# mgholamikn/PoseGen

Measured on AMD Instinct MI355X. Metric: rendered rays/sec (512x512, 64 samples/ray), higher is better.
Workload: dtype bf16

## Files before the change

posegen_amd/csrc/pg_api.hip:

```cpp
#include <hip/hip_runtime.h>

#include <cstdarg>
#include <cstdio>
#include <cstdlib>
#include <chrono>
#include <cstring>
#include <algorithm>
#include <mutex>
#include <thread>
#include <new>
#include <utility>
#include <vector>

#include "../../include/posegen_hip.h"
#include "pg_device.h"
#include "pg_handle.h"
#include "pg_pack.h"

extern "C" {
int pg_launch_eval16(const pgd::EvalArgs* a, int fp16, int framecode, int grid, void* stream);
int pg_launch_eval16r(const pgd::EvalArgs* a, int fp16, int framecode, int onchip, int grid, void* stream);
int pg_launch_ray_records(const pgd::RecArgs* a, int fp16, int framecode, int n_cu, void* stream);
int pg_eval16_points_per_pass(void);
int pg_eval16_wgs_per_cu(void);
// ... 130 lines not shown
    }
}

enum Form {
    F_DIRECT16,
    F_REC16,
    F_ONCHIP16,
    F_C2,
    F_COMP_DIRECT,
    F_COMP_REC,
    F_COMP_ONCHIP,
    F_KMAJOR,
    F_COUNT
};

struct Switches {
    bool view_fact = true;
    bool comp_kernel = true;
    bool comp_rec = true;
    bool evalc2 = true;
    int onchip = PG_ONCHIP_AUTO;
};
const Switches& switches() {
    static const Switches sw = [] {
        auto off = [](const char* name) { const char* e = std::getenv(name); return e && e[0] == '0'; };
        Switches s;
        s.view_fact = !off("POSEGEN_VIEW_FACT");
        s.comp_kernel = !off("POSEGEN_COMP_KERNEL");
        s.comp_rec = !off("POSEGEN_COMP_REC");
        s.evalc2 = !off("POSEGEN_EVALC2");
        const char* e = std::getenv("POSEGEN_ONCHIP");
        s.onchip = e && e[0] == '0' ? PG_ONCHIP_RECORDS : e && e[0] == '2' ? PG_ONCHIP_ALWAYS : PG_ONCHIP_AUTO;
        return s;
    }();
    return sw;
}

struct CallFacts {
    int prec;
    int S;
    long long pose_stride;
    bool fc;
    bool points, pnoise;
    bool dbg; int dbg_stage;
    int onchip_mode;
};

// ... 273 lines not shown
    a.S = S;
    a.n_codes = ns.n_codes;
    a.tau_v = h->tau[0];
    a.tau_d = h->tau[1];
    a.dbg_stage = dbg_stage;
    a.far_skip = h->far_skip ? 1 : 0;
    const int pts = fi.points_per_pass();
    if (!points && S < pts / (MAXR - 1))
        return pg_fail(h, PG_EINVAL, "N_samples=%d too small: the fused kernel needs >= %d samples per ray", S, pts / (MAXR - 1));
    const long long iters = (a.n_points + pts - 1) / pts;
    a.n_iters = (int)iters;
    static const long long wg_cap = [] { const char* e = std::getenv("POSEGEN_MAX_WG"); return e ? std::atoll(e) : 0ll; }();
    long long max_wg = (long long)h->n_cu * fi.wgs_per_cu();
    if (wg_cap > 0 && wg_cap < max_wg) max_wg = wg_cap;
    const int grid = (int)(iters < max_wg ? iters : max_wg);
    hipEvent_t e0 = nullptr, e1 = nullptr;
    auto get = [&](hipEvent_t& ev) {
        if (!h->ev_free.empty()) { ev = h->ev_free.back(); h->ev_free.pop_back(); return hipSuccess; }
        return hipEventCreate(&ev);
    };
    if (y_bytes) {
        pgd::RecArgs ra{};
        ra.rays = rays; ra.skts = skts; ra.cams = cams; ra.codes = a.codes; ra.wy = a.wy;
        ra.rec_ab = const_cast<float*>(a.rec_ab); ra.rec_y = const_cast<uint8_t*>(a.rec_y);
        ra.pose_stride = pose_stride; ra.n_rays = (int)n; ra.n_codes = ns.n_codes;
        ra.z = z; ra.S = S;
        hipEvent_t x0 = nullptr, x1 = nullptr;
        if (h->profiling) { PG_HIP(h, get(x0)); PG_HIP(h, get(x1)); PG_HIP(h, hipEventRecord(x0, static_cast<hipStream_t>(stream))); }
        const int er = form == F_COMP_REC ? pg_launch_ray_records_c(&ra, fc, h->n_cu, stream) : pg_launch_ray_records(&ra, prec == PG_PREC_FP16, fc, h->n_cu, stream);
        if (h->profiling) {
// ... 483 lines not shown

int pg_debug_widen_views(const float* view_w, int64_t rows, int64_t cols, int framecode_ch, float* out, int64_t cap,
                         int64_t* out_n) {
    if (!view_w) return pg_fail(nullptr, PG_EINVAL, "pg_debug_widen_views: null argument");
    if (framecode_ch != 0 && framecode_ch != FC_CH) return pg_fail(nullptr, PG_EINVAL, "pg_debug_widen_views: frame code 0 or 16");
    if (rows != VW || cols != W + CH_D0 + framecode_ch)
        return pg_fail(nullptr, PG_EINVAL, "pg_debug_widen_views: view weight [%lld,%lld], expected [%d,%d]", (long long)rows,
                       (long long)cols, VW, W + CH_D0 + framecode_ch);
    const int64_t need = (int64_t)VW * (W + CH_D + framecode_ch);
    if (out_n) *out_n = need;
    if (out) {
        if (cap < need) return pg_fail(nullptr, PG_EINVAL, "pg_debug_widen_views: buffer too small");
        widen_view_w(view_w, framecode_ch, out);
    }
    return PG_OK;
}

int pg_debug_pack_vy(const float* const* tensors, const int64_t* shapes, int n_tensors, int framecode_ch,
                     int precision, uint8_t* out, int64_t cap, int64_t* out_bytes) {
    if (!tensors || !shapes || n_tensors != 24) return pg_fail(nullptr, PG_EINVAL, "pg_debug_pack_vy: need 24 tensors");
    NetState ns;
    host_copy(ns, tensors, shapes, framecode_ch);
    pg_config cfg{};
    cfg.framecode_ch = framecode_ch;
    std::vector<uint8_t> vy;
    if (precision == PG_PREC_FP16C) {
        std::vector<float> f;
        pgpack::pack_vyc(tensors_of(ns, cfg), framecode_ch > 0, f);
        vy.resize(f.size() * sizeof(float));
        std::memcpy(vy.data(), f.data(), vy.size());
// ... 796 lines not shown
```

posegen_amd/csrc/pg_device.h:

```cpp
#pragma once
#include <hip/hip_runtime.h>

#include <atomic>

#include "pg_program.h"

namespace pgd {
using namespace pgl;

typedef __attribute__((ext_vector_type(8))) __bf16 bf16x8;
typedef __attribute__((ext_vector_type(8))) _Float16 f16x8;
typedef __attribute__((ext_vector_type(16))) float f32x16;

struct EvalArgs {
    const float* rays;
    const float* z;
    const float* pts;
    const float* pnoise;
    const float* skts;
    const float* cams;
    const float* codes;
    const uint8_t* wstream;
    const uint8_t* wy;
    const float* rec_ab;
    const uint8_t* rec_y;
    const float* bias;
    const float* cutoff;
    float* raw;
    float* dbg;
    long long pose_stride;
    long long n_points;
    int n_rays;
    int S;
    int n_codes;
    int n_iters;
    float tau_v, tau_d;
    int dbg_stage;
    int far_skip;
};

struct RecArgs {
    const float* rays;
    const float* skts;
    const float* cams;
    const float* codes;
    const uint8_t* wy;
    float* rec_ab;
    uint8_t* rec_y;
    const float* z;
    long long pose_stride;
    int n_rays;
    int n_codes;
    int S;
};

template <const int (&P)[24]>
__device__ __forceinline__ int perm_dev(int s) {
    constexpr unsigned long long lo = [] { unsigned long long v = 0; for (int i = 0; i < 12; ++i) v |= (unsigned long long)P[i] << (5 * i); return v; }();
    constexpr unsigned long long hi = [] { unsigned long long v = 0; for (int i = 0; i < 12; ++i) v |= (unsigned long long)P[12 + i] << (5 * i); return v; }();
    return (int)(((s < 12 ? lo : hi) >> (5 * (s < 12 ? s : s - 12))) & 31);
}
__device__ __forceinline__ int slot_joint_dev(int s) { return perm_dev<PERM16>(s); }
__device__ __forceinline__ int slotc_joint_dev(int s) { return perm_dev<PERMC>(s); }

inline hipError_t ensure_lds_attr(const void* fn, int bytes, std::atomic<unsigned long long>& done) {
    int dev = 0;
    hipError_t e = hipGetDevice(&dev);
    if (e != hipSuccess) return e;
// ... 379 lines not shown
```

posegen_amd/csrc/pg_eval16r.hip:

```cpp
#ifndef PG_PREFETCH
#define PG_PREFETCH 1
#endif
#ifndef PG_PIPE_H
#define PG_PIPE_H 4
#endif
#include <type_traits>

#include "pg_eval16_common.h"

#ifndef PG_REC_POLICY
#define PG_REC_POLICY ""
#endif

namespace pgd {

typedef __attribute__((ext_vector_type(4))) float f32x4;

template <typename V> struct Op16;
template <> struct Op16<bf16x8> {
    static __device__ __forceinline__ f32x4 mfma(bf16x8 a, bf16x8 b, f32x4 c) {
        return __builtin_amdgcn_mfma_f32_16x16x32_bf16(a, b, c, 0, 0, 0);
    }
};
template <> struct Op16<f16x8> {
// ... 270 lines not shown
    const float tlv = a.tau_v * 1.4426950408889634f, tld = a.tau_d * 1.4426950408889634f;
    if (tid < 48) cut[tid] = -a.cutoff[(tid < J ? 0 : J) + slot_joint_dev(tid < J ? tid : tid - J)] * (tid < J ? tlv : tld);
    else if (tid < 72) {
        const int jt = slot_joint_dev(tid - 48);
        const float far = fmaxf(a.cutoff[jt] + 24.0f / tlv, a.cutoff[J + jt] + 24.0f / tld);
        cut[tid] = far * far;
    }
    if (OC) {
        if (!PP) for (int i = tid; i < J * 12; i += NTHR) reinterpret_cast<float*>(smem + LDSR_SK)[i] = a.skts[slot_joint_dev(i / 12) * 16 + i % 12];
        for (int i = tid; i < MAXR_F * REC_Y_BYTES / 16; i += NTHR) reinterpret_cast<uint4*>(smem + LDSR_Y)[i] = make_uint4(0u, 0u, 0u, 0u);
    }
#if defined(PG_YOUNG_PRIO)
    if (wave >= NWAVE / 2) __builtin_amdgcn_s_setprio(PG_YOUNG_PRIO);
#endif
    const unsigned bbase = lds_addr_of(bias) + 16 * g;
    const long long step = (long long)PTS * gridDim.x;
    const int dq = __builtin_amdgcn_readfirstlane((int)(step / a.S)), dr = __builtin_amdgcn_readfirstlane((int)(step % a.S));
    long long p0 = (long long)blockIdx.x * PTS;
    int r0 = __builtin_amdgcn_readfirstlane((int)(p0 / a.S));
    int off0 = __builtin_amdgcn_readfirstlane((int)(p0 - (long long)r0 * a.S));
    if (OC) {
        lds_barrier();
        if (tid < MAXR_F * J) {
            const int k = tid / J, sl = tid - k * J;
            const long long ray = min((long long)r0 + k, (long long)a.n_rays - 1);
            const float* skr = PP ? a.skts + ray * a.pose_stride + slot_joint_dev(sl) * 16 : sk_lds + sl * 12;
            ab_row(skr, a.rays + ray * 11, a.z[ray * a.S], a.z[ray * a.S + a.S - 1],
                   reinterpret_cast<float4*>(smem + LDSR_AB + k * REC_AB_BYTES + sl * 32));
        }
    } else if ((int)blockIdx.x < a.n_iters && wave < LDS_AB_BYTES / 1024)
        dma_piece(rec_ab + (long long)r0 * REC_AB_BYTES + wave * 1024, lds0 + LDSR_AB + wave * 1024, lane16);
    if (OC && FC) {
        const float* ytab = reinterpret_cast<const float*>(a.wy);
        for (int idx = tid; idx < MAXR_F * VW; idx += NTHR) {
            const int k = idx / VW, o = idx - k * VW;
// ... 17 lines not shown
#endif
    st.start((uint32_t)gmask);

    float nx_z[2] = {0.0f, 0.0f};
#define PG_PREFETCH_Z(itn)                                                                         \
    do {                                                                                           \
        const long long p0n_ = (long long)(itn) * PTS + wave * 32 + col;                           \
        nx_z[0] = a.z[min(p0n_, a.n_points - 1)];                                                  \
        nx_z[1] = a.z[min(p0n_ + 16, a.n_points - 1)];                                             \
    } while (0)
    if ((int)blockIdx.x < a.n_iters) PG_PREFETCH_Z(blockIdx.x);

#if defined(PG_STAMPS)
    unsigned long long stamps[12];
#endif
    for (int it = blockIdx.x; it < a.n_iters; it += gridDim.x) {
        PG_STAMP(0);
        int lane_p = lane;
        asm volatile("" : "+v"(lane_p));
        const int g_p = lane_p >> 4;
        const int last = (int)min((long long)PTS - 1, a.n_points - 1 - p0);
        const int S1 = a.S, S2 = 2 * a.S, S3 = 3 * a.S, S4 = 4 * a.S;
        auto ray_of = [&](int t) { return (t >= S1) + (t >= S2) + (t >= S3) + (t >= S4); };
        const int nrm1 = ray_of(off0 + last);
        int myr[2];
        float zz[2];
        const float* abp[2];
#pragma unroll
        for (int c = 0; c < 2; ++c) {
            const int i = wave * 32 + 16 * c + col;
            myr[c] = min(ray_of(off0 + i), nrm1);
            zz[c] = nx_z[c];
            abp[c] = opaque_ptr(reinterpret_cast<const float*>(smem + LDSR_AB + abuf * LDS_AB_BYTES + myr[c] * REC_AB_BYTES) + JG * g_p * 8);
        }
        const int itn = min(it + (int)gridDim.x, a.n_iters - 1);
        int off0n = off0 + dr, r0n = r0 + dq;
        if (off0n >= a.S) { off0n -= a.S; ++r0n; }
        const float* cutd = opaque_ptr(cut + J + JG * g_p);
        const QFromAB q0{abp[0], zz[0]}, q1{abp[1], zz[1]};
        float cutv[JG];
#pragma unroll
        for (int jj = 0; jj < JG; ++jj) cutv[jj] = cut[JG * g_p + jj];
        int farmask = 0;
#if !defined(PG_NO_FAR_SKIP)
        {
            const float* far2 = opaque_ptr(cut + 2 * J + JG * g_p);
#pragma unroll
            for (int jj = 0; jj < JG; ++jj) {
                float ax, ay, az, bx, by, bz;
                q0(jj, ax, ay, az);
                q1(jj, bx, by, bz);
                const bool near = fminf(ax * ax + ay * ay + az * az, bx * bx + by * by + bz * bz) < far2[jj];
                if (__builtin_amdgcn_ballot_w64(near) == 0ull) farmask |= 1 << jj;
            }
            farmask = __builtin_amdgcn_readfirstlane(a.far_skip ? farmask : 0);
        }
#endif
        if (CNT && lane == 0) {
            if (wave == 0) { atomicAdd(reinterpret_cast<unsigned*>(a.dbg), 1u); atomicAdd(reinterpret_cast<unsigned*>(a.dbg) + 1, (unsigned)__builtin_popcount(gmask)); }
            atomicAdd(reinterpret_cast<unsigned*>(a.dbg) + 2, (unsigned)__builtin_popcount(farmask));
        }
        auto fetch_records = [&]() {
            if (OC) {
                const long long rn = min((long long)r0n, (long long)a.n_rays - 1);
                if (wave == 0) dma_dwords(a.rays, (uint32_t)(min(rn * 11 + lane_p, (long long)a.n_rays * 11 - 1) * 4), lds0 + LDSR_STAGE);
                else if (wave == 1) {
                    const long long ray = min(rn + min(lane_p >> 1, MAXR_F - 1), (long long)a.n_rays - 1);
                    dma_dwords(a.z, (uint32_t)((ray * a.S + ((lane_p & 1) ? a.S - 1 : 0)) * 4), lds0 + LDSR_STAGE + 256);
                } else if (FC && wave == 2 && a.cams)
                    dma_dwords(a.cams, (uint32_t)(min(rn + min(lane_p, MAXR_F - 1), (long long)a.n_rays - 1) * 4), lds0 + LDSR_STAGE + 512);
                return;
// ... 77 lines not shown
                    if (u == PG_R_BIAS_AT && o + 1 < NT16) bp.fetch(o + 1);
                }
            }
            x_segment16<V>(acc, st, abp[0], abp[1], zz[0], zz[1], cutv, tlv, farmask, gmask, [] {});
#pragma unroll
            for (int u = 0; u < HU16; ++u)
#pragma unroll
                for (int c = 0; c < 2; ++c) fb[u][c] = relu_pack16<V>(acc[2 * u][c], acc[2 * u + 1][c], true);
        }
        PG_STAMP(4);
        hidden_layer16<V>(fb, fa, st, bbase, BS_LAYER0 + 6 * NT16, C_L6);
        hidden_layer16<V>(fa, fb, st, bbase, BS_LAYER0 + 7 * NT16, C_L6 + CH);
        PG_STAMP(5);
        int gmask_n = 0;
#if !defined(PG_NO_FAR_SKIP)
        gmask_n = pass_far_mask(smem + LDSR_AB + (abuf ^ 1) * LDS_AB_BYTES, rays_of_pass(p0 + step, off0n),
                                opaque_ptr(cut + 2 * J + JG * g_p), g_p, lane_p & 15);
        if (!a.far_skip) gmask_n = 0;
#endif
        st.nx_mask = (uint32_t)gmask_n;
        float sigma[2];
        V fg[NTV16 / 2][2];
        APipe<V> pv;
        {
            f32x4 vacc[NTV16][2];
            constexpr int TAV = pgp::R::U_AV;
            static_assert(BS_VIEWF == BS_ALPHA + 1 && BS_RGB == BS_VIEWF + NTV16, "alpha, view and rgb bias tiles are consecutive");
            BiasPipe bp(bbase, BS_ALPHA);
            bp.fetch(0);
#pragma unroll
            for (int o = 0; o < NTV16 + 1; ++o) {
// ... 35 lines not shown
            bp.fetch(0);
#pragma unroll
            for (int u = 0; u < pgp::R::U_RGB; ++u) {
                const V av = next_a_cont<V, pgp::R::U_RGB, PG_PIPE_H, pgp::R::U_AV % UPC>(pr, st, u);
                if (u == 0) c0 = c1 = bp.take();
                c0 = Op16<V>::mfma(av, fg[u][0], c0);
                c1 = Op16<V>::mfma(av, fg[u][1], c1);
            }
        }
        if (g == 0) {
            const int i = wave * 32 + col;
            if (i <= last) *reinterpret_cast<float4*>(a.raw + (p0 + i) * 4) = make_float4(c0[0], c0[1], c0[2], sigma[0]);
            if (i + 16 <= last) *reinterpret_cast<float4*>(a.raw + (p0 + i + 16) * 4) = make_float4(c1[0], c1[1], c1[2], sigma[1]);
        }
        abuf ^= 1;
        p0 += step; r0 = r0n; off0 = off0n;
        gmask = gmask_n;
        PG_STAMP(8);
#if defined(PG_STAMPS)
        if (a.dbg && a.dbg_stage == 99 && lane == 0 && it < 64) {
            for (int k = 0; k < 9; ++k) reinterpret_cast<unsigned long long*>(a.dbg)[((long long)it * NWAVE + wave) * 16 + k] = stamps[k];
            reinterpret_cast<unsigned long long*>(a.dbg)[((long long)it * NWAVE + wave) * 16 + 9] = st.t_vm;
            reinterpret_cast<unsigned long long*>(a.dbg)[((long long)it * NWAVE + wave) * 16 + 10] = st.t_bar;
            st.t_vm = 0; st.t_bar = 0;
        }
#endif
    }
    st.drain();
}

template <typename V, bool FC, bool TAPS, bool OC, bool CNT = false, bool PP = false>
static hipError_t launch_eval16r(const EvalArgs& a, int grid, hipStream_t stream) {
    auto k = eval16r_kernel<V, FC, TAPS, OC, CNT, PP>;
    constexpr int lds = OC ? LDSR_TOTAL_OC : LDSR_TOTAL;
    static std::atomic<unsigned long long> attr_done{0};
    const hipError_t ae = ensure_lds_attr(reinterpret_cast<const void*>(k), lds, attr_done);
    if (ae != hipSuccess) return ae;
    hipLaunchKernelGGL(k, dim3(grid), dim3(NTHR), lds, stream, a);
    return hipGetLastError();
}

template <typename V>
static hipError_t dispatch_eval16r(const EvalArgs& a, int framecode, int onchip, int grid, hipStream_t s) {
// ... 21 lines not shown
```

posegen_amd/csrc/pg_evalc.hip:

```cpp
#include <type_traits>

#include "pg_comp.h"

#ifndef PG_REC_POLICY
#define PG_REC_POLICY " nt"
#endif

namespace pgd {

constexpr int NWAVE_C = 4;
constexpr int NTHR_C = NWAVE_C * 64;
constexpr int PTS_C = NWAVE_C * 32;
using StreamC = Stream<NWAVE_C, pgp::C::NCHUNK, NWAVE_C>;
using StreamCR = Stream<NWAVE_C, pgp::C::NCHUNK_R, NWAVE_C, pgp::C::NPAIRJ, 0, pgp::C::C_L5XR>;
using StreamCRO = Stream<NWAVE_C, pgp::C::NCHUNK_OC, NWAVE_C, pgp::C::NPAIRJ, 0, pgp::C::C_L5XR_OC, pgp::C::C_YC>;
static_assert(StreamCRO::plain_ok(27) && StreamCRO::plain_ok(63) && !StreamCRO::plain_ok(64) && !StreamCRO::plain_ok(70) && StreamCRO::plain_ok(82) &&
              StreamCRO::plain_ok(100) && !StreamCRO::plain_ok(101) && !StreamCRO::plain_ok(12) && !StreamCRO::plain_ok(5) && StreamCRO::plain_ok(26), "on-chip stream: L1 .. L5h, L6 .. rgb");
static_assert(StreamCR::plain_ok(15) && StreamCR::plain_ok(51) && !StreamCR::plain_ok(52) && StreamCR::plain_ok(70) && StreamCR::plain_ok(88) &&
              !StreamCR::plain_ok(89), "record stream");
#ifndef PG_NSC
#define PG_NSC 5
#endif
constexpr int NSC = PG_NSC;
constexpr int LDS_TOTAL_C = LDS_RTAB + MAXR_C * SLOTC_FLOATS * 4;
// ... 464 lines not shown
        if (tid < 48) cut[tid] = -a.cutoff[(tid < J ? 0 : J) + slotc_joint_dev(tid < J ? tid : tid - J)] * (tid < J ? tlv : tld);
        else if (tid < 72) {
            const int jt = slotc_joint_dev(tid - 48);
            const float far = fmaxf(a.cutoff[jt] + 24.0f / tlv, a.cutoff[J + jt] + 24.0f / tld);
            cut[tid] = far * far;
        }
    } else if (tid < 48) cut[tid] = -a.cutoff[tid] * (tid < J ? tlv : tld);
    if (OC) {
        for (int i = tid; i < J * 12; i += NTHR_C) reinterpret_cast<float*>(smem + LDSO_SK)[i] = a.skts[slotc_joint_dev(i / 12) * 16 + i % 12];
        for (int i = tid; i < MAXR_CR * RECC_Y_BYTES / 16; i += NTHR_C) reinterpret_cast<uint4*>(smem + LDSO_Y)[i] = make_uint4(0u, 0u, 0u, 0u);
    }
    float s129 = (float)COMP_S;
    asm volatile("" : "+s"(s129));
    if (!REC) st.start();

    const long long step = (long long)PTS_C * gridDim.x;
    int dq = 0, dr = 0, r0 = 0, off0 = 0, abuf = 0;
    long long p0 = (long long)blockIdx.x * PTS_C;
    const uint8_t* rec_ab = reinterpret_cast<const uint8_t*>(a.rec_ab);
    if (REC) {
        dq = __builtin_amdgcn_readfirstlane((int)(step / a.S)); dr = __builtin_amdgcn_readfirstlane((int)(step % a.S));
        r0 = __builtin_amdgcn_readfirstlane((int)(p0 / a.S));
        off0 = __builtin_amdgcn_readfirstlane((int)(p0 - (long long)r0 * a.S));
        if (OC) {
            lds_barrier();
            if (tid < MAXR_CR * J) {
                const int k = tid / J, sl = tid - k * J;
                const long long ray = min((long long)r0 + k, (long long)a.n_rays - 1);
                ab_row(sk_lds + sl * 12, a.rays + ray * 11, a.z[ray * a.S], a.z[ray * a.S + a.S - 1],
                       reinterpret_cast<float4*>(smem + LDSC_AB + k * REC_AB_BYTES + sl * 32));
            }
        } else if ((int)blockIdx.x < a.n_iters && wave < LDS_ABC_BYTES / 1024)
            dma_piece_c(rec_ab + (long long)r0 * REC_AB_BYTES + wave * 1024, lds0 + LDSC_AB + wave * 1024, lane16);
        asm volatile("s_waitcnt vmcnt(0)" ::: "memory");
        lds_barrier();
    }
    auto rays_of_pass = [&](long long p0_, int off0_) {
        const int last_ = (int)max(0ll, min((long long)PTS_C - 1, a.n_points - 1 - p0_));
// ... 2 lines not shown
    };
    int gmask = 0;
    if (REC) {
#if !defined(PG_NO_FAR_SKIP)
        gmask = pass_far_mask_c(smem + LDSC_AB, rays_of_pass(p0, off0), cut + 2 * J + JH * h, h, pt);
        if (!a.far_skip) gmask = 0;
#endif
        st.start((uint32_t)gmask);
    }
    float nx_z = 0.0f;
    if (REC && (int)blockIdx.x < a.n_iters) nx_z = a.z[min(p0 + wave * 32 + pt, a.n_points - 1)];

#if defined(PG_STAMPS)
    unsigned long long stamps[14];
#endif
    for (int it = blockIdx.x; it < a.n_iters; it += gridDim.x) {
        PG_STAMP(0);
#if defined(PG_STAMPS)
        { unsigned long long t_; asm volatile("s_memrealtime %0\n\ts_waitcnt lgkmcnt(0)" : "=s"(t_) :: "memory"); stamps[10] = t_; }
#endif
        const long long gp = p0 + wave * 32 + pt;
        const bool valid = gp < a.n_points;
        const long long gpc = valid ? gp : a.n_points - 1;
        int myr, r0n = 0, off0n = 0, nrm1 = 0;
        const float* slot = nullptr;
        const float* ab;
        const float* tab = nullptr;
        if (REC) {
            const int last = (int)min((long long)PTS_C - 1, a.n_points - 1 - p0);
            const int S1 = a.S, S2 = 2 * a.S;
            const int tl_ = off0 + last, ti = off0 + wave * 32 + pt;
            nrm1 = (tl_ >= S1) + (tl_ >= S2);
            myr = min((ti >= S1) + (ti >= S2), nrm1);
            ab = opaque_ptr(reinterpret_cast<const float*>(smem + LDSC_AB + abuf * ABSZ + myr * REC_AB_BYTES) + JH * h * 8);
            off0n = off0 + dr; r0n = r0 + dq;
            if (off0n >= a.S) { off0n -= a.S; ++r0n; }
        } else {
            const long long plast = min(p0 + PTS_C - 1, a.n_points - 1);
            r0 = (int)(p0 / a.S);
            const int nr = (int)(plast / a.S) - r0 + 1;
            lds_barrier();
            ray_table_c<FC>(a, rtab, r0, nr);
            lds_barrier();
            myr = (int)(gpc / a.S) - r0;
            slot = rtab + myr * SLOTC_FLOATS;
            ab = opaque_ptr(slot + SLOTC_AB + JH * h * 8);
            tab = opaque_ptr(slot + SLOTC_DTAB + h * DSEQ);
        }
        const float* cutv = opaque_ptr(cut + JH * h);
        const float* cutd = opaque_ptr(cut + J + JH * h);
        const float zz = REC ? nx_z : a.z[gpc];
// ... 97 lines not shown
        PG_STAMP(5);
#pragma unroll
        for (int o = 0; o < NT; ++o) accA[o] = load_bias(bias, BT_LAYER0 + 6 * NT + o, h);
        segment_c<NT, HU, true>(accA, st, srcB, s129, C_L6);
#pragma unroll
        for (int o = 0; o < NT; ++o) accB[o] = load_bias(bias, BT_LAYER0 + 7 * NT + o, h);
        segment_c<NT, HU, true>(accB, st, srcA, s129, C_L6 + CH);
        if (TAPS && a.dbg && a.dbg_stage == 7 && valid) {
#pragma unroll
            for (int i = 0; i < HSEQ; ++i) a.dbg[gp * W + hseq_channel(i, h)] = fmaxf(accB[i >> 4][i & 15], 0.0f);
        }
        PG_STAMP(6);
        int gmask_n = 0;
        if (REC) {
#if !defined(PG_NO_FAR_SKIP)
            gmask_n = pass_far_mask_c(smem + LDSC_AB + (abuf ^ 1) * ABSZ, rays_of_pass(p0 + step, off0n),
                                      opaque_ptr(cut + 2 * J + JH * h), h, pt);
            if (!a.far_skip) gmask_n = 0;
#endif
            st.nx_mask = (uint32_t)gmask_n;
        }
        f32x16 av[NTV + 1];
        av[0] = load_bias(bias, TB_ALPHA, h);
#pragma unroll
        for (int o = 0; o < NTV; ++o) av[1 + o] = load_bias(bias, TB_VIEWF + o, h);
        segment_c<NTV + 1, HU, true>(av, st, srcB, s129, C_AV);
        const float sigma = av[0][0];
        PG_STAMP(7);
        {
            float wd[JH];
#pragma unroll
// ... 39 lines not shown
            } else {
                const float* code = slot + SLOTC_CODE + 8 * h;
                auto srcD = [&](int u, int e) {
                    if (u == pgp::C::DU) return code[e];
                    const int k = u < JH * 3 ? u / 3 : (8 * (u - JH * 3) + e) / 3;
                    return k < JH ? tab[u * 8 + e] * wd[k] : 0.0f;
                };
                segment_c<NTV, pgp::C::DU + (FC ? 1 : 0), false>(av + 1, st, srcD, s129);
            }
        }
        if (TAPS && a.dbg && a.dbg_stage == 9 && valid) {
#pragma unroll
            for (int i = 0; i < VW / 2; ++i) a.dbg[gp * W + hseq_channel(i, h)] = fmaxf(av[1 + (i >> 4)][i & 15], 0.0f);
        }
        PG_STAMP(8);
        if (REC) nx_z = a.z[min(p0 + step + wave * 32 + pt, a.n_points - 1)];
        f32x16 accr = load_bias(bias, TB_RGB, h);
        auto srcV = [&](int u, int e) { return av[1 + (u >> 1)][8 * (u & 1) + e]; };
#if defined(PG_ABL_NORGB)
        { PairPipe<NSC> pq; st.enter_split(); for (int i = 0; i < ST::PER; ++i) piece_c(pq, st, i); asm volatile("" :: "v"(av[1][0]), "v"(av[2][0]), "v"(av[3][0]), "v"(av[4][0])); }
#else
        segment_c<1, HU / 2, true>(&accr, st, srcV, s129);
#endif
#if defined(PG_STAMPS_RGB)
        PG_STAMP(9);
#endif
#if defined(PG_ABL_NOSTORE)
        asm volatile("" :: "v"(accr[0]), "v"(accr[1]), "v"(accr[2]), "v"(sigma));
#else
        if (valid && h == 0)
            *reinterpret_cast<float4*>(a.raw + gp * 4) = make_float4(accr[0], accr[1], accr[2], sigma);
#endif
        if (REC) { abuf ^= 1; r0 = r0n; off0 = off0n; gmask = gmask_n; }
        p0 += step;
#if !defined(PG_STAMPS_RGB)
        PG_STAMP(9);
#endif
#if defined(PG_STAMPS)
        { unsigned long long t_; asm volatile("s_memrealtime %0\n\ts_waitcnt lgkmcnt(0)" : "=s"(t_) :: "memory"); stamps[11] = t_; }
        if (a.dbg && a.dbg_stage == 99 && lane == 0 && it < 64) {
            reinterpret_cast<unsigned long long*>(a.dbg)[((long long)it * 8 + wave) * 16 + 12] = stamps[10];
            reinterpret_cast<unsigned long long*>(a.dbg)[((long long)it * 8 + wave) * 16 + 13] = stamps[11];
            for (int k = 0; k < 10; ++k) reinterpret_cast<unsigned long long*>(a.dbg)[((long long)it * 8 + wave) * 16 + k] = stamps[k];
            reinterpret_cast<unsigned long long*>(a.dbg)[((long long)it * 8 + wave) * 16 + 10] = st.t_vm;
            reinterpret_cast<unsigned long long*>(a.dbg)[((long long)it * 8 + wave) * 16 + 11] = st.t_bar;
            st.t_vm = 0; st.t_bar = 0;
        }
#endif
    }
// ... 33 lines not shown
```

posegen_amd/csrc/pg_evalc2.hip:

```cpp
#include <type_traits>

#include "pg_comp.h"

namespace pgd {
namespace c2 {
namespace TT = pgp::T;
typedef __attribute__((ext_vector_type(4))) float f32x4;

constexpr int NTHR2 = TT::NW * 64;
constexpr int NX = 5;
constexpr int L_REG = 0;
constexpr int UNIT_LDS = TT::NCT * 2 * 1024;
constexpr int L_REG_BYTES = HU16 * UNIT_LDS;
constexpr int L_BIAS = L_REG + L_REG_BYTES;
constexpr int L_CUT = L_BIAS + BIAS16_FLOATS * 4;
constexpr int L_ALPHA = L_CUT + 72 * 4;
constexpr int L_RGB = L_ALPHA + TT::SMALL_ALPHA;
constexpr int L_AB = L_RGB + TT::SMALL_RGB;
constexpr int L_ABSZ = TT::MAXR * REC_AB_BYTES;
constexpr int L_CMASK = L_AB + 2 * L_ABSZ;
constexpr int L_SK = L_CMASK + 64;
constexpr int L_TOTAL = L_SK + J * 12 * 4;
static_assert(L_BIAS % 16 == 0 && L_CUT % 16 == 0 && L_ALPHA % 16 == 0 && L_RGB % 16 == 0 && L_AB % 16 == 0 && L_CMASK % 16 == 0 && L_SK % 16 == 0,
              "LDS alignment");
// ... 256 lines not shown
    for (int i = tid; i < BIAS16_FLOATS; i += NTHR2) bias[i] = a.bias[i];
    const float tlv = a.tau_v * 1.4426950408889634f, tld = a.tau_d * 1.4426950408889634f;
    if (tid < 48) cut[tid] = -a.cutoff[(tid < J ? 0 : J) + slot_joint_dev(tid < J ? tid : tid - J)] * (tid < J ? tlv : tld);
    else if (tid < 72) {
        const int jt = slot_joint_dev(tid - 48);
        const float far = fmaxf(a.cutoff[jt] + 24.0f / tlv, a.cutoff[J + jt] + 24.0f / tld);
        cut[tid] = far * far;
    }
    for (int i = tid; i < (TT::SMALL_ALPHA + TT::SMALL_RGB) / 16; i += NTHR2)
        reinterpret_cast<uint4*>(smem + L_ALPHA)[i] = reinterpret_cast<const uint4*>(wbase + TT::OFF_SMALL)[i];
    if (!PP)
        for (int i = tid; i < J * 12; i += NTHR2) reinterpret_cast<float*>(smem + L_SK)[i] = a.skts[slot_joint_dev(i / 12) * 16 + i % 12];
    float s129 = (float)COMP_S;
    asm volatile("" : "+s"(s129));

    const long long step = (long long)TT::PTS * gridDim.x;
    const int dq = __builtin_amdgcn_readfirstlane((int)(step / a.S)), dr = __builtin_amdgcn_readfirstlane((int)(step % a.S));
    long long p0 = (long long)blockIdx.x * TT::PTS;
    int r0 = __builtin_amdgcn_readfirstlane((int)(p0 / a.S));
    int off0 = __builtin_amdgcn_readfirstlane((int)(p0 - (long long)r0 * a.S));
    const int S1 = a.S, S2 = 2 * a.S, S3 = 3 * a.S, S4 = 4 * a.S;
    auto ray_of = [&](int t) { return (t >= S1) + (t >= S2) + (t >= S3) + (t >= S4); };
    auto load_ray_item = [&](int item, int rr, float* ray6, float& z0, float& z1, float* sk12) {
        const int k = item / J, sl = item - k * J;
        const long long ray = min((long long)rr + k, (long long)a.n_rays - 1);
#pragma unroll
        for (int e = 0; e < 6; ++e) ray6[e] = a.rays[ray * 11 + e];
        z0 = a.z[ray * a.S];
        z1 = a.z[ray * a.S + a.S - 1];
        if (PP) {
            const float4* skp = reinterpret_cast<const float4*>(a.skts + ray * a.pose_stride + slot_joint_dev(sl) * 16);
            const float4 r0_ = skp[0], r1_ = skp[1], r2_ = skp[2];
            sk12[0] = r0_.x; sk12[1] = r0_.y; sk12[2] = r0_.z; sk12[3] = r0_.w;
            sk12[4] = r1_.x; sk12[5] = r1_.y; sk12[6] = r1_.z; sk12[7] = r1_.w;
            sk12[8] = r2_.x; sk12[9] = r2_.y; sk12[10] = r2_.z; sk12[11] = r2_.w;
// ... 15 lines not shown
    if ((int)blockIdx.x < a.n_iters) nx_z = a.z[min(p0 + 16 * wave + col, a.n_points - 1)];
    lds_barrier();

    const bool count_skips = a.dbg != nullptr && a.dbg_stage == 97;
    unsigned n_cnt[3] = {0u, 0u, 0u};
#if defined(PG_C2_YOUNG_PRIO)
    if (wave >= 4) __builtin_amdgcn_s_setprio(PG_C2_YOUNG_PRIO);
#endif
    const uint8_t* wx_wave = wbase + wave * TT::KBLK;
    WPair W[4];
    ASet X[NX];

#if defined(PG_STAMPS)
    unsigned long long stamp_acc[12] = {}, stamp_prev = 0;
#endif
    for (int it = blockIdx.x; it < a.n_iters; it += gridDim.x) {
#if defined(PG_STAMPS)
        { unsigned long long t_; asm volatile("s_memtime %0\n\ts_waitcnt lgkmcnt(0)" : "=s"(t_) :: "memory"); stamp_prev = t_; }
#endif
        int lane_p;
        asm volatile("v_mbcnt_lo_u32_b32 %0, -1, 0\n\tv_mbcnt_hi_u32_b32 %0, -1, %0" : "=v"(lane_p));
        const uint8_t* wx_p = wx_wave;
        const uint8_t* wb_p = wbase;
        asm volatile("" : "+s"(wx_p), "+s"(wb_p));
        const int g_p = lane_p >> 4, col_p = lane_p & 15;
        const unsigned lane16 = (unsigned)lane_p * 16u;
        const unsigned hb_lo = lds0 + L_REG + lane16;
        uint8_t* const lane_reg = smem + L_REG + lane_p * 16;
        const int last = (int)min((long long)TT::PTS - 1, a.n_points - 1 - p0);
        const int nrm1 = ray_of(off0 + last);
        const int i_pt = 16 * wave + col_p;
        const int myr = min(ray_of(off0 + i_pt), nrm1);
        const float zz = nx_z;
        const float* abp = opaque_ptr(reinterpret_cast<const float*>(smem + L_AB + abuf * L_ABSZ + myr * REC_AB_BYTES) + JG * g_p * 8);
        int off0n = off0 + dr, r0n = r0 + dq;
        if (off0n >= a.S) { off0n -= a.S; ++r0n; }
        auto local = [&](int jj, float& qx, float& qy, float& qz) {
            const float4 lo = *reinterpret_cast<const float4*>(abp + jj * 8);
            const float4 hi = *reinterpret_cast<const float4*>(abp + jj * 8 + 4);
            qx = fmaf(zz, hi.x, lo.x); qy = fmaf(zz, hi.y, lo.y); qz = fmaf(zz, hi.z, lo.z);
        };

        int wm = 0;
#if !defined(PG_NO_FAR_SKIP)
        {
            const float* far2 = cut + 2 * J + JG * g_p;
#pragma unroll
            for (int jj = 0; jj < JG; ++jj) {
                float qx, qy, qz;
                local(jj, qx, qy, qz);
                if (__builtin_amdgcn_ballot_w64(qx * qx + qy * qy + qz * qz < far2[jj]) == 0ull) wm |= 1 << jj;
// ... 425 lines not shown
            a128 b0 = ld128(wp), b1 = ld128(wp + 1024), b2 = ld128(wp + 2048), b3 = ld128(wp + 3072);
            const uint8_t* ya = lane_reg + L_Y + ra * L_YRAY + (2 * v4) * 2048;
            const uint8_t* yb = lane_reg + L_Y + rb * L_YRAY + (2 * v4) * 2048;
            a128 a0 = ld128(ya), a1 = ld128(ya + 1024), a2 = ld128(ya + 2048), a3 = ld128(ya + 3072);
            a128 e0 = ld128(yb), e1 = ld128(yb + 1024), e2 = ld128(yb + 2048), e3 = ld128(yb + 3072);
            pin4(b0, b1, b2, b3); pin4(a0, a1, a2, a3); pin4(e0, e1, e2, e3);
            av[0][cc] = mma(a0, b0, av[0][cc]);
            av[1][cc] = mma(a2, b0, av[1][cc]);
            av[0][cc] = mma(a1, b1, av[0][cc]);
            av[1][cc] = mma(a3, b1, av[1][cc]);
            av[0][cc] = mma(e0, b2, av[0][cc]);
            av[1][cc] = mma(e2, b2, av[1][cc]);
            av[0][cc] = mma(e1, b3, av[0][cc]);
            av[1][cc] = mma(e3, b3, av[1][cc]);
        }
        nx_z = a.z[min(p0 + step + 16 * wave + col_p, a.n_points - 1)];
        a128 rgA[VW / 32][2];
        {
            const uint8_t* rp = smem + L_RGB + ((lane_p & 15) < 3 ? (3 * g_p + (lane_p & 15)) * 16 : 12 * 16);
#pragma unroll
            for (int u = 0; u < VW / 32; ++u) {
                rgA[u][0] = ld128(rp + (2 * u) * TT::RGB_STRIDE);
                rgA[u][1] = ld128(rp + (2 * u + 1) * TT::RGB_STRIDE);
            }
        }
        lds_barrier();
#pragma unroll
        for (int cc = 0; cc < 4; ++cc) {
            unsigned h[4], x[4];
            const float v[8] = {av[0][cc][0], av[0][cc][1], av[0][cc][2], av[0][cc][3], av[1][cc][0], av[1][cc][1], av[1][cc][2], av[1][cc][3]};
            conv4<true>(v, h, x, s129);
// ... 8 lines not shown
            a128 g0 = ld128(gp), g1 = ld128(gp + 1024), g2 = ld128(gp + UNIT_LDS), g3 = ld128(gp + UNIT_LDS + 1024);
            a128 g4 = ld128(gp + 2 * UNIT_LDS), g5 = ld128(gp + 2 * UNIT_LDS + 1024), g6 = ld128(gp + 3 * UNIT_LDS), g7 = ld128(gp + 3 * UNIT_LDS + 1024);
            pin4(g0, g1, g2, g3); pin4(g4, g5, g6, g7);
            c3 = mma(rgA[0][0], g0, c3); c3 = mma(rgA[0][1], g1, c3);
            c3 = mma(rgA[1][0], g2, c3); c3 = mma(rgA[1][1], g3, c3);
            c3 = mma(rgA[2][0], g4, c3); c3 = mma(rgA[2][1], g5, c3);
            c3 = mma(rgA[3][0], g6, c3); c3 = mma(rgA[3][1], g7, c3);
        }
        {
            int ipt3 = 16 * wave + col_p;
            asm volatile("" : "+v"(ipt3));
            if (g_p == 0 && ipt3 <= last)
                *reinterpret_cast<float4*>(a.raw + (p0 + ipt3) * 4) = make_float4(c3[0], c3[1], c3[2], al[0]);
        }
        abuf ^= 1;
        p0 += step; r0 = r0n; off0 = off0n;
        C2_STAMP(10);
#if defined(PG_STAMPS)
        stamp_acc[11] += 1;
#endif
    }
#if defined(PG_STAMPS)
    if (a.dbg && a.dbg_stage == 99 && lane == 0)
        for (int k = 0; k < 12; ++k) reinterpret_cast<unsigned long long*>(a.dbg)[((long long)blockIdx.x * TT::NW + wave) * 16 + k] = stamp_acc[k];
#endif
    if (count_skips && tid == 0)
        for (int k = 0; k < 3; ++k) atomicAdd(reinterpret_cast<unsigned*>(a.dbg) + k, n_cnt[k]);
    asm volatile("s_waitcnt vmcnt(0)" ::: "memory");
}

template <bool FC, bool PP>
// ... 22 lines not shown
```

Baseline: 8.313 million.

## Replace fixed grid-stride pass order with rotated walk across workgroups

Introduces a PassWalk iterator that assigns passes to workgroups using a per-round rotation (rho, default 99 mod grid) instead of a plain grid-stride, and uses it in the eval16r, evalc and evalc2 fused kernels. The intent is to spread far-skip-heavy or cheap passes more evenly across workgroups so that load imbalance and tail effects shrink. It also adds a host-side checker that the walk covers every pass exactly once, plus optional timing stamps. The walk adds a little per-iteration scalar arithmetic, and changing the pass order may affect cache locality of the per-ray records.

```diff
diff --git a/posegen_amd/csrc/pg_api.hip b/posegen_amd/csrc/pg_api.hip
--- a/posegen_amd/csrc/pg_api.hip
+++ b/posegen_amd/csrc/pg_api.hip
@@ -168,12 +168,14 @@
     F_COUNT
 };
 
+constexpr int PASS_WALK_RHO = 99;
 struct Switches {
     bool view_fact = true;
     bool comp_kernel = true;
     bool comp_rec = true;
     bool evalc2 = true;
     int onchip = PG_ONCHIP_AUTO;
+    int pass_walk = PASS_WALK_RHO;
 };
 const Switches& switches() {
     static const Switches sw = [] {
@@ -185,6 +187,7 @@
         s.evalc2 = !off("POSEGEN_EVALC2");
         const char* e = std::getenv("POSEGEN_ONCHIP");
         s.onchip = e && e[0] == '0' ? PG_ONCHIP_RECORDS : e && e[0] == '2' ? PG_ONCHIP_ALWAYS : PG_ONCHIP_AUTO;
+        if (const char* w = std::getenv("POSEGEN_PASS_WALK")) s.pass_walk = std::max(0, std::atoi(w));
         return s;
     }();
     return sw;
@@ -488,6 +491,7 @@
     long long max_wg = (long long)h->n_cu * fi.wgs_per_cu();
     if (wg_cap > 0 && wg_cap < max_wg) max_wg = wg_cap;
     const int grid = (int)(iters < max_wg ? iters : max_wg);
+    a.walk_rho = switches().pass_walk % grid;
     hipEvent_t e0 = nullptr, e1 = nullptr;
     auto get = [&](hipEvent_t& ev) {
         if (!h->ev_free.empty()) { ev = h->ev_free.back(); h->ev_free.pop_back(); return hipSuccess; }
@@ -1001,6 +1005,24 @@
         widen_view_w(view_w, framecode_ch, out);
     }
     return PG_OK;
+}
+
+extern "C" long long pg_debug_pass_walk(long long n_rays, int S, int pts, int G, int rho) {
+    if (n_rays <= 0 || S <= 0 || pts <= 0 || G <= 0 || rho < 0 || rho >= G) return -1;
+    const long long n_iters = (n_rays * S + pts - 1) / pts;
+    std::vector<uint8_t> taken((size_t)n_iters, 0);
+    long long bad = 0;
+    for (int b = 0; b < G; ++b) {
+        int prev = -1;
+        for (pgd::PassWalk w(S, pts, b, G, rho); w.it < n_iters; w.advance(), w.peek()) {
+            const long long p0 = (long long)w.it * pts;
+            if (w.p0 != p0 || w.r0 != p0 / S || w.off0 != p0 % S || w.it <= prev || w.it / G != w.itn / G - 1 || taken[(size_t)w.it]) ++bad;
+            taken[(size_t)w.it] = 1;
+            prev = w.it;
+        }
+    }
+    for (long long i = 0; i < n_iters; ++i) bad += !taken[(size_t)i];
+    return bad;
 }
 
 int pg_debug_pack_vy(const float* const* tensors, const int64_t* shapes, int n_tensors, int framecode_ch,
diff --git a/posegen_amd/csrc/pg_device.h b/posegen_amd/csrc/pg_device.h
--- a/posegen_amd/csrc/pg_device.h
+++ b/posegen_amd/csrc/pg_device.h
@@ -37,6 +37,7 @@
     float tau_v, tau_d;
     int dbg_stage;
     int far_skip;
+    int walk_rho;
 };
 
 struct RecArgs {
@@ -52,6 +53,44 @@
     int n_rays;
     int n_codes;
     int S;
+};
+
+struct PassWalk {
+    int S, G, rho, pts;
+    int dq[2], dr[2];
+    int it, c;
+    long long p0;
+    int r0, off0;
+    int itn, cn, r0n, off0n;
+    long long p0n;
+    static __host__ __device__ __forceinline__ int uni(int v) {
+#if defined(__HIP_DEVICE_COMPILE__)
+        return __builtin_amdgcn_readfirstlane(v);
+#else
+        return v;
+#endif
+    }
+    __host__ __device__ __forceinline__ PassWalk(int S_, int pts_, int b, int G_, int rho_) : S(S_), G(G_), rho(rho_), pts(pts_) {
+        const long long s0 = (long long)pts * (G + rho), s1 = (long long)pts * rho;
+        dq[0] = uni((int)(s0 / S)); dr[0] = uni((int)(s0 % S));
+        dq[1] = uni((int)(s1 / S)); dr[1] = uni((int)(s1 % S));
+        it = c = b;
+        p0 = (long long)b * pts;
+        r0 = uni((int)(p0 / S));
+        off0 = uni((int)(p0 - (long long)r0 * S));
+        peek();
+    }
+    __host__ __device__ __forceinline__ void peek() {
+        const int wrap = c + rho >= G ? 1 : 0;
+        const int di = wrap ? rho : G + rho;
+        itn = it + di;
+        cn = c + rho - (wrap ? G : 0);
+        p0n = p0 + (long long)di * pts;
+        off0n = off0 + dr[wrap];
+        r0n = r0 + dq[wrap];
+        if (off0n >= S) { off0n -= S; ++r0n; }
+    }
+    __host__ __device__ __forceinline__ void advance() { it = itn; c = cn; p0 = p0n; r0 = r0n; off0 = off0n; }
 };
 
 template <const int (&P)[24]>
diff --git a/posegen_amd/csrc/pg_eval16r.hip b/posegen_amd/csrc/pg_eval16r.hip
--- a/posegen_amd/csrc/pg_eval16r.hip
+++ b/posegen_amd/csrc/pg_eval16r.hip
@@ -308,11 +308,9 @@
     if (wave >= NWAVE / 2) __builtin_amdgcn_s_setprio(PG_YOUNG_PRIO);
 #endif
     const unsigned bbase = lds_addr_of(bias) + 16 * g;
-    const long long step = (long long)PTS * gridDim.x;
-    const int dq = __builtin_amdgcn_readfirstlane((int)(step / a.S)), dr = __builtin_amdgcn_readfirstlane((int)(step % a.S));
-    long long p0 = (long long)blockIdx.x * PTS;
-    int r0 = __builtin_amdgcn_readfirstlane((int)(p0 / a.S));
-    int off0 = __builtin_amdgcn_readfirstlane((int)(p0 - (long long)r0 * a.S));
+    PassWalk pw(a.S, PTS, (int)blockIdx.x, (int)gridDim.x, a.walk_rho);
+    long long p0 = pw.p0;
+    int r0 = pw.r0, off0 = pw.off0;
     if (OC) {
         lds_barrier();
         if (tid < MAXR_F * J) {
@@ -360,7 +358,12 @@
 #if defined(PG_STAMPS)
     unsigned long long stamps[12];
 #endif
-    for (int it = blockIdx.x; it < a.n_iters; it += gridDim.x) {
+#if defined(PG_WALK_STAMPS)
+    unsigned long long walk_t0;
+    asm volatile("s_memtime %0\n\ts_waitcnt lgkmcnt(0)" : "=s"(walk_t0) :: "memory");
+    unsigned walk_passes = 0, walk_limbs = 0;
+#endif
+    for (int it = pw.it; it < a.n_iters; it = pw.it) {
         PG_STAMP(0);
         int lane_p = lane;
         asm volatile("" : "+v"(lane_p));
@@ -379,9 +382,8 @@
             zz[c] = nx_z[c];
             abp[c] = opaque_ptr(reinterpret_cast<const float*>(smem + LDSR_AB + abuf * LDS_AB_BYTES + myr[c] * REC_AB_BYTES) + JG * g_p * 8);
         }
-        const int itn = min(it + (int)gridDim.x, a.n_iters - 1);
-        int off0n = off0 + dr, r0n = r0 + dq;
-        if (off0n >= a.S) { off0n -= a.S; ++r0n; }
+        const int itn = min(pw.itn, a.n_iters - 1);
+        const int off0n = pw.off0n, r0n = pw.r0n;
         const float* cutd = opaque_ptr(cut + J + JG * g_p);
         const QFromAB q0{abp[0], zz[0]}, q1{abp[1], zz[1]};
         float cutv[JG];
@@ -401,6 +403,9 @@
             }
             farmask = __builtin_amdgcn_readfirstlane(a.far_skip ? farmask : 0);
         }
+#endif
+#if defined(PG_WALK_STAMPS)
+        walk_passes += 1; walk_limbs += (unsigned)__builtin_popcount(~gmask & 63);
 #endif
         if (CNT && lane == 0) {
             if (wave == 0) { atomicAdd(reinterpret_cast<unsigned*>(a.dbg), 1u); atomicAdd(reinterpret_cast<unsigned*>(a.dbg) + 1, (unsigned)__builtin_popcount(gmask)); }
@@ -508,7 +513,7 @@
         PG_STAMP(5);
         int gmask_n = 0;
 #if !defined(PG_NO_FAR_SKIP)
-        gmask_n = pass_far_mask(smem + LDSR_AB + (abuf ^ 1) * LDS_AB_BYTES, rays_of_pass(p0 + step, off0n),
+        gmask_n = pass_far_mask(smem + LDSR_AB + (abuf ^ 1) * LDS_AB_BYTES, rays_of_pass(pw.p0n, off0n),
                                 opaque_ptr(cut + 2 * J + JG * g_p), g_p, lane_p & 15);
         if (!a.far_skip) gmask_n = 0;
 #endif
@@ -574,7 +579,8 @@
             if (i + 16 <= last) *reinterpret_cast<float4*>(a.raw + (p0 + i + 16) * 4) = make_float4(c1[0], c1[1], c1[2], sigma[1]);
         }
         abuf ^= 1;
-        p0 += step; r0 = r0n; off0 = off0n;
+        pw.advance(); pw.peek();
+        p0 = pw.p0; r0 = pw.r0; off0 = pw.off0;
         gmask = gmask_n;
         PG_STAMP(8);
 #if defined(PG_STAMPS)
@@ -587,6 +593,16 @@
 #endif
     }
     st.drain();
+#if defined(PG_WALK_STAMPS)
+    if (CNT && tid == 0) {
+        unsigned long long walk_t1;
+        asm volatile("s_memtime %0\n\ts_waitcnt lgkmcnt(0)" : "=s"(walk_t1) :: "memory");
+        unsigned* rec = reinterpret_cast<unsigned*>(a.dbg) + 16 + 8 * blockIdx.x;
+        rec[0] = (unsigned)walk_t0; rec[1] = (unsigned)(walk_t0 >> 32);
+        rec[2] = (unsigned)walk_t1; rec[3] = (unsigned)(walk_t1 >> 32);
+        rec[4] = walk_passes; rec[5] = walk_limbs;
+    }
+#endif
 }
 
 template <typename V, bool FC, bool TAPS, bool OC, bool CNT = false, bool PP = false>
diff --git a/posegen_amd/csrc/pg_evalc.hip b/posegen_amd/csrc/pg_evalc.hip
--- a/posegen_amd/csrc/pg_evalc.hip
+++ b/posegen_amd/csrc/pg_evalc.hip
@@ -502,14 +502,11 @@
     asm volatile("" : "+s"(s129));
     if (!REC) st.start();
 
-    const long long step = (long long)PTS_C * gridDim.x;
-    int dq = 0, dr = 0, r0 = 0, off0 = 0, abuf = 0;
-    long long p0 = (long long)blockIdx.x * PTS_C;
+    PassWalk pw(a.S, PTS_C, (int)blockIdx.x, (int)gridDim.x, REC ? a.walk_rho : 0);
+    int r0 = pw.r0, off0 = pw.off0, abuf = 0;
+    long long p0 = pw.p0;
     const uint8_t* rec_ab = reinterpret_cast<const uint8_t*>(a.rec_ab);
     if (REC) {
-        dq = __builtin_amdgcn_readfirstlane((int)(step / a.S)); dr = __builtin_amdgcn_readfirstlane((int)(step % a.S));
-        r0 = __builtin_amdgcn_readfirstlane((int)(p0 / a.S));
-        off0 = __builtin_amdgcn_readfirstlane((int)(p0 - (long long)r0 * a.S));
         if (OC) {
             lds_barrier();
             if (tid < MAXR_CR * J) {
@@ -542,7 +539,7 @@
 #if defined(PG_STAMPS)
     unsigned long long stamps[14];
 #endif
-    for (int it = blockIdx.x; it < a.n_iters; it += gridDim.x) {
+    for (int it = pw.it; it < a.n_iters; it = pw.it) {
         PG_STAMP(0);
 #if defined(PG_STAMPS)
         { unsigned long long t_; asm volatile("s_memrealtime %0\n\ts_waitcnt lgkmcnt(0)" : "=s"(t_) :: "memory"); stamps[10] = t_; }
@@ -561,8 +558,7 @@
             nrm1 = (tl_ >= S1) + (tl_ >= S2);
             myr = min((ti >= S1) + (ti >= S2), nrm1);
             ab = opaque_ptr(reinterpret_cast<const float*>(smem + LDSC_AB + abuf * ABSZ + myr * REC_AB_BYTES) + JH * h * 8);
-            off0n = off0 + dr; r0n = r0 + dq;
-            if (off0n >= a.S) { off0n -= a.S; ++r0n; }
+            off0n = pw.off0n; r0n = pw.r0n;
         } else {
             const long long plast = min(p0 + PTS_C - 1, a.n_points - 1);
             r0 = (int)(p0 / a.S);
@@ -690,7 +686,7 @@
         int gmask_n = 0;
         if (REC) {
 #if !defined(PG_NO_FAR_SKIP)
-            gmask_n = pass_far_mask_c(smem + LDSC_AB + (abuf ^ 1) * ABSZ, rays_of_pass(p0 + step, off0n),
+            gmask_n = pass_far_mask_c(smem + LDSC_AB + (abuf ^ 1) * ABSZ, rays_of_pass(pw.p0n, off0n),
                                       opaque_ptr(cut + 2 * J + JH * h), h, pt);
             if (!a.far_skip) gmask_n = 0;
 #endif
@@ -760,7 +756,7 @@
             for (int i = 0; i < VW / 2; ++i) a.dbg[gp * W + hseq_channel(i, h)] = fmaxf(av[1 + (i >> 4)][i & 15], 0.0f);
         }
         PG_STAMP(8);
-        if (REC) nx_z = a.z[min(p0 + step + wave * 32 + pt, a.n_points - 1)];
+        if (REC) nx_z = a.z[min(pw.p0n + wave * 32 + pt, a.n_points - 1)];
         f32x16 accr = load_bias(bias, TB_RGB, h);
         auto srcV = [&](int u, int e) { return av[1 + (u >> 1)][8 * (u & 1) + e]; };
 #if defined(PG_ABL_NORGB)
@@ -778,7 +774,8 @@
             *reinterpret_cast<float4*>(a.raw + gp * 4) = make_float4(accr[0], accr[1], accr[2], sigma);
 #endif
         if (REC) { abuf ^= 1; r0 = r0n; off0 = off0n; gmask = gmask_n; }
-        p0 += step;
+        pw.advance(); pw.peek();
+        p0 = pw.p0;
 #if !defined(PG_STAMPS_RGB)
         PG_STAMP(9);
 #endif
diff --git a/posegen_amd/csrc/pg_evalc2.hip b/posegen_amd/csrc/pg_evalc2.hip
--- a/posegen_amd/csrc/pg_evalc2.hip
+++ b/posegen_amd/csrc/pg_evalc2.hip
@@ -294,11 +294,9 @@
     float s129 = (float)COMP_S;
     asm volatile("" : "+s"(s129));
 
-    const long long step = (long long)TT::PTS * gridDim.x;
-    const int dq = __builtin_amdgcn_readfirstlane((int)(step / a.S)), dr = __builtin_amdgcn_readfirstlane((int)(step % a.S));
-    long long p0 = (long long)blockIdx.x * TT::PTS;
-    int r0 = __builtin_amdgcn_readfirstlane((int)(p0 / a.S));
-    int off0 = __builtin_amdgcn_readfirstlane((int)(p0 - (long long)r0 * a.S));
+    PassWalk pw(a.S, TT::PTS, (int)blockIdx.x, (int)gridDim.x, a.walk_rho);
+    long long p0 = pw.p0;
+    int r0 = pw.r0, off0 = pw.off0;
     const int S1 = a.S, S2 = 2 * a.S, S3 = 3 * a.S, S4 = 4 * a.S;
     auto ray_of = [&](int t) { return (t >= S1) + (t >= S2) + (t >= S3) + (t >= S4); };
     auto load_ray_item = [&](int item, int rr, float* ray6, float& z0, float& z1, float* sk12) {
@@ -344,7 +342,7 @@
 #if defined(PG_STAMPS)
     unsigned long long stamp_acc[12] = {}, stamp_prev = 0;
 #endif
-    for (int it = blockIdx.x; it < a.n_iters; it += gridDim.x) {
+    for (; pw.it < a.n_iters; pw.advance(), pw.peek()) {
 #if defined(PG_STAMPS)
         { unsigned long long t_; asm volatile("s_memtime %0\n\ts_waitcnt lgkmcnt(0)" : "=s"(t_) :: "memory"); stamp_prev = t_; }
 #endif
@@ -363,8 +361,7 @@
         const int myr = min(ray_of(off0 + i_pt), nrm1);
         const float zz = nx_z;
         const float* abp = opaque_ptr(reinterpret_cast<const float*>(smem + L_AB + abuf * L_ABSZ + myr * REC_AB_BYTES) + JG * g_p * 8);
-        int off0n = off0 + dr, r0n = r0 + dq;
-        if (off0n >= a.S) { off0n -= a.S; ++r0n; }
+        const int off0n = pw.off0n, r0n = pw.r0n;
         auto local = [&](int jj, float& qx, float& qy, float& qz) {
             const float4 lo = *reinterpret_cast<const float4*>(abp + jj * 8);
             const float4 hi = *reinterpret_cast<const float4*>(abp + jj * 8 + 4);
@@ -820,7 +817,7 @@
             av[0][cc] = mma(e1, b3, av[0][cc]);
             av[1][cc] = mma(e3, b3, av[1][cc]);
         }
-        nx_z = a.z[min(p0 + step + 16 * wave + col_p, a.n_points - 1)];
+        nx_z = a.z[min(pw.p0n + 16 * wave + col_p, a.n_points - 1)];
         a128 rgA[VW / 32][2];
         {
             const uint8_t* rp = smem + L_RGB + ((lane_p & 15) < 3 ? (3 * g_p + (lane_p & 15)) * 16 : 12 * 16);
@@ -859,7 +856,7 @@
                 *reinterpret_cast<float4*>(a.raw + (p0 + ipt3) * 4) = make_float4(c3[0], c3[1], c3[2], al[0]);
         }
         abuf ^= 1;
-        p0 += step; r0 = r0n; off0 = off0n;
+        p0 = pw.p0n; r0 = r0n; off0 = off0n;
         C2_STAMP(10);
 #if defined(PG_STAMPS)
         stamp_acc[11] += 1;
```

After: 8.918 million, median of 6. +7.3%, better.
